# PSeitz/veloci

Hardware: AMD Instinct MI355X
Metric: queries/sec, 3-term AND on 100M-doc index (p50 latency and HBM fraction alongside) (higher is better)
Workload: dtype u32 doc ids + f16->f32 scores

## Files before the change

veloci_amd/csrc/scan_probe.hip:

```cpp
#include <hip/hip_runtime.h>
#include <hip/hip_fp16.h>

#include "device_types.hpp"
#include "kernel_common.hpp"
#include "kernels.hpp"
#include "probe_common.hpp"

namespace vq {

#ifdef VQ_STAMP
__device__ unsigned long long g_probe_stamp[16];
#define PS_INIT                                                      \
    unsigned long long _st0 = __builtin_amdgcn_s_memtime();          \
    const unsigned long long _t0 = _st0;                             \
    const unsigned long long _r0 = __builtin_amdgcn_s_memrealtime(); \
    unsigned long long _acc[16] = {0};
#define PS_AT(k)                                                \
    {                                                           \
        unsigned long long _st1 = __builtin_amdgcn_s_memtime(); \
        _acc[k] += _st1 - _st0;                                 \
        _st0 = _st1;                                            \
    }
#define PS_COUNT(k) _acc[k] += 1ull;
#define PS_FLUSH                                                                                             \
    _acc[14] = __builtin_amdgcn_s_memtime() - _t0;                        \
    _acc[15] = __builtin_amdgcn_s_memrealtime() - _r0;                \
    if (threadIdx.x == 0) {                                                                                  \
        _Pragma("unroll") for (int _k = 0; _k < 16; ++_k) if (_acc[_k]) atomicAdd(&g_probe_stamp[_k], _acc[_k]); \
    }
void debug_read_probe_stamps(unsigned long long* out, int reset) {
    (void)hipMemcpyFromSymbol(out, HIP_SYMBOL(g_probe_stamp), sizeof(unsigned long long) * 16);
    if (reset) {
        unsigned long long z[16] = {0};
        (void)hipMemcpyToSymbol(HIP_SYMBOL(g_probe_stamp), z, sizeof z);
    }
}
#else
#define PS_INIT
#define PS_AT(k)
#define PS_COUNT(k)
#define PS_FLUSH
#endif

constexpr uint32_t kPMaxR = 2;
constexpr uint32_t kPU = 256;
static_assert(kPU >= 256, "a round of 256 postings must fit the empty queue");
constexpr uint32_t kPR = 128;
constexpr uint32_t kPLdsShape = 8;
constexpr uint32_t kPLdsU = kPLdsShape + 24;
constexpr uint32_t kPLdsR = kPLdsU + kPU;
__host__ __device__ constexpr uint32_t probe_lds_tile(uint32_t nd) { return kPLdsR + (2 + nd) * kPR; }
__host__ __device__ constexpr uint32_t probe_lds_arr(uint32_t nd, uint32_t nb) { return probe_lds_tile(nd) + nb * (kPTW + kPRk); }
size_t scan_probe_lds_bytes(uint32_t cand_cap, uint32_t nd, uint32_t na, uint32_t arr_slot) {
    return (size_t)(probe_lds_arr(nd, nd - na) + na * arr_slot + 2 * cand_cap) * 4 + 16;
}

template <uint32_t ND, uint32_t NA, bool OR = false>
__device__ __forceinline__ void probe_body(const uint8_t* __restrict__ blob, const uint32_t span, const uint32_t q, const uint32_t cand_cap, const uint32_t arr_slot,
                                           unsigned long long* __restrict__ span_keys, unsigned long long* __restrict__ num_hits) {
    extern __shared__ __attribute__((aligned(16))) uint32_t lds[];
    const uint32_t lane = threadIdx.x;
    const VQ_CONST QHeader* H = as_const<QHeader>(blob);
    const VQ_CONST DList* gl = as_const<DList>(blob + H->off_lists);
    const VQ_CONST DOp* gops = as_const<DOp>(blob + H->off_ops);
    const VQ_CONST DProbe* P = as_const<DProbe>(blob + H->off_simple2);
    const uint32_t sflags = H->simple_flags;
    const uint32_t top_k = H->top_k;
    constexpr uint32_t n = ND + 1u;
    constexpr uint32_t NB = ND - NA;
    constexpr uint32_t NB1 = NB ? NB : 1u, NA1 = NA ? NA : 1u;
    PS_INIT

    unsigned long long* thr = reinterpret_cast<unsigned long long*>(lds);
    uint32_t* cand_n = lds + 2;
    uint32_t* sh = lds + kPLdsShape;
    uint32_t* uq = lds + kPLdsU;
    uint32_t* rq = lds + kPLdsR;
    uint32_t* tile = lds + probe_lds_tile(ND);
    uint32_t* rank = tile + NB * kPTW;
    uint32_t* arr = lds + probe_lds_arr(ND, NB);
    unsigned long long* cand = reinterpret_cast<unsigned long long*>(arr + NA * arr_slot);
    unsigned long long* const gthr = reinterpret_cast<unsigned long long*>(const_cast<uint8_t*>(blob) + offsetof(QHeader, gthr));
    CandState cs{cand, cand_n, thr, cand_cap, gthr};
    cs.upper = H->key_upper;
    uint32_t* const stat = H->stat_off ? lds + 4 : nullptr;
    uint8_t* const pool = H->off_pool ? const_cast<uint8_t*>(blob) + H->off_pool : nullptr;

    const uint32_t* ccov = nullptr;
    const uint32_t* cgdir = nullptr;
    const uint32_t* d_bitmap[NB1];
    const uint32_t* d_rank[NB1];
    const uint16_t* d_arr[NA1];
    const uint32_t* d_agd[NA1];
    {
        const uint32_t ck = (uint32_t)__ffs((int)((sflags >> 8) & 0xFu)) - 1u;
        const uint32_t am = (sflags >> 12) & 0xFu;
        uint32_t role_of[4] = {0u, 0u, 0u, 0u};
        uint32_t ib = 0, ia = NB;
#pragma unroll
        for (uint32_t k = 0; k < n; ++k) {
            const VQ_CONST DList& d = gl[gops[k].list_begin];
            if (k == ck) {
                ccov = P->leaf[k].cov32;
                cgdir = P->leaf[k].gdir;
                if (lane == 0) {
                    sh[kShCts] = __float_as_uint(d.term_score);
                    sh[kShPrunable] = (d.term_score > 0.0f && d.max_raw < 0x7C00u) ? 1u : 0u;
                }
            } else {
                const bool is_arr = ((am >> k) & 1u) != 0u;
                const uint32_t role = is_arr ? ia : ib;
#pragma unroll
                for (uint32_t j = 0; j < NB; ++j)
                    if (!is_arr && j == role) {
                        d_bitmap[j] = d.bitmap;
                        d_rank[j] = d.rank_dir;
                    }
#pragma unroll
                for (uint32_t a = 0; a < NA; ++a)
                    if (is_arr && NB + a == role) {
                        d_arr[a] = P->leaf[k].arr16;
                        d_agd[a] = P->leaf[k].gdir;
                    }
                if (lane == 0) {
                    const uint16_t mr = d.max_raw;
                    sh[kShTs + role] = __float_as_uint(d.term_score);
                    sh[kShVmax + role] = (d.term_score > 0.0f && mr < 0x7C00u) ? __float_as_uint(posting_value(d.term_score, mr)) : 0x7F800000u;
                    reinterpret_cast<unsigned long long*>(sh + kShScores)[role] = is_arr ? (unsigned long long)(uintptr_t)P->leaf[k].cov32 : (unsigned long long)(uintptr_t)d.scores;
                }
                role_of[k] = 1u + role;
                if (is_arr) ++ia;
                else ++ib;
            }
        }
        const KOp root(gops + n);
#pragma unroll
        for (uint32_t j = 0; j < n; ++j) {
            const uint32_t k = OR ? j : root.and_order(j);
            if (lane == 0) sh[kShSrc + j] = k == 0u ? role_of[0] : k == 1u ? role_of[1] : k == 2u ? role_of[2] : role_of[3];
        }
    }

    const uint32_t n_spans = H->n_spans;
    const unsigned long long range = (unsigned long long)(H->doc_hi - H->doc_lo);
    const uint32_t span_lo = span == 0 ? H->doc_lo : ((H->doc_lo + (uint32_t)(range * span / n_spans)) & ~(kPT - 1u));
    const uint32_t span_hi = span + 1 == n_spans ? H->doc_hi : ((H->doc_lo + (uint32_t)(range * (span + 1) / n_spans)) & ~(kPT - 1u));
    const uint32_t bitmap_base = H->bitmap_base;
    const uint32_t keys_base = H->keys_base;

    if (lane == 0) {
        *thr = __hip_atomic_load(gthr, __ATOMIC_RELAXED, __HIP_MEMORY_SCOPE_AGENT);
        *cand_n = 0;
        lds[4] = 0u;
    }
    __syncthreads();
    unsigned long long thr_seen = *thr;
    uint32_t raw_min = 0u;
    constexpr uint32_t kMasks = OR ? (1u << ND) : 1u;
    uint32_t rmin[kMasks];
    auto take_raw_min = [&](const float thr_f) {
        if (OR) {
#pragma unroll
            for (uint32_t m = 0; m < kMasks; ++m) rmin[m] = probe_raw_min<ND>(sh, thr_f, lane, m);
        } else raw_min = probe_raw_min<ND>(sh, thr_f, lane);
    };
    take_raw_min(__uint_as_float(unorder_f32((uint32_t)(thr_seen >> 32))));

    const u32x4 kSent = u32x4{0xFFFFFFFFu, 0xFFFFFFFFu, 0xFFFFFFFFu, 0xFFFFFFFFu};
    const VQ_GLOBAL u32x4* cc4 = as_global(reinterpret_cast<const u32x4*>(ccov));

    uint32_t un = 0, rn = 0;
    uint32_t ucnt = 0;
    unsigned long long hits = 0;
    unsigned long long g_prev = 0ull;

    const uint32_t t_first = (span_lo - bitmap_base) >> kProbeTileShift;
    const uint32_t t_end = span_hi > span_lo ? ((span_hi - 1u - bitmap_base) >> kProbeTileShift) + 1u : t_first;
    uint32_t dir_base = t_first;
    auto load_dir = [&](const uint32_t* g) { return as_global(g)[dir_base + lane < t_end ? dir_base + lane : t_end]; };
    uint32_t dirv = load_dir(cgdir);
    uint32_t adv[NA1];
#pragma unroll
    for (uint32_t a = 0; a < NA; ++a) adv[a] = load_dir(d_agd[a]);
    auto dir_at = [&](const uint32_t v, const uint32_t tt) { return (uint32_t)__builtin_amdgcn_readlane((int)v, (int)(tt - dir_base)); };

    u32x4 wk[ND][kPNV];
    uint32_t rk[NB1];
    u32x4 nid[kPMaxR], cid[kPMaxR];
#pragma unroll
    for (uint32_t r = 0; r < kPMaxR; ++r) nid[r] = cid[r] = kSent;
    uint32_t pf_rounds = 0, pf_v0 = 0, pf_v1 = 0;
    uint32_t na_g0[NA1], na_nv[NA1];
    uint32_t a_g0[NA1], a_cnt[NA1];
#pragma unroll
    for (uint32_t a = 0; a < NA1; ++a) na_g0[a] = na_nv[a] = a_g0[a] = a_cnt[a] = 0u;
    auto issue_tile = [&](const uint32_t tt, const uint32_t g0, const uint32_t g1) {
        pf_rounds = (g1 - g0 + 31u) >> 5;
        pf_v0 = g0 * 2u;
        pf_v1 = g1 * 2u;
        if (OR || pf_rounds) {
#pragma unroll
            for (uint32_t i = 0; i < NB; ++i) {
                const VQ_GLOBAL u32x4* gb = as_global(reinterpret_cast<const u32x4*>(d_bitmap[i] + (size_t)tt * kPTW));
#pragma unroll
                for (uint32_t h = 0; h < kPNV; ++h) wk[i][h] = gb[h * 64u + lane];
                rk[i] = as_global(d_rank[i])[tt * kPRk + lane];
            }
#pragma unroll
            for (uint32_t a = 0; a < NA; ++a) {
                const VQ_GLOBAL u32x4* ga = as_global(reinterpret_cast<const u32x4*>(d_arr[a]) + na_g0[a]);
#pragma unroll
                for (uint32_t h = 0; h < kPNV; ++h)
                    if (h * 64u + lane < na_nv[a]) wk[NB + a][h] = ga[h * 64u + lane];
            }
#pragma unroll
            for (uint32_t r = 0; r < kPMaxR; ++r) {
                const uint32_t v = pf_v0 + r * 64u + lane;
                nid[r] = kSent;
                if (r < pf_rounds && v < pf_v1) nid[r] = cc4[v];
            }
        }
    };

    uint32_t tile_lo = 0;
    uint32_t f_stage = 0;
    uint32_t f_doc = 0, f_idx[ND];
    float f_vc = 0.0f, f_vd[ND];
    uint16_t f_r = 0;
    bool f_alive = false;
#pragma unroll
    for (uint32_t i = 0; i < ND; ++i) {
        f_idx[i] = 0u;
        f_vd[i] = 0.0f;
    }
    uint32_t rhead = 0;
    uint32_t tiles_since_merge = 8;
    auto push_keys = [&](const unsigned long long key, bool pending, const bool final) {
        if (wballot(pending)) {
            while (true) {
                if (pending) {
                    if (key > *thr) {
                        uint32_t pos = atomicAdd(cs.n, 1u);
                        if (pos < cs.cap) {
                            cs.cand[pos] = key;
                            pending = false;
                        }
                    } else pending = false;
                }
                probe_lds_fence();
                if (!wballot(pending)) break;
                cand_prune(cs, top_k);
            }
            if (pool && (tiles_since_merge >= 8u || final)) {
                PS_COUNT(13)
                tiles_since_merge = 0;
                probe_pool_merge<true>(cs, top_k, pool, lane);
            }
            const unsigned long long tn = *thr;
            if ((uint32_t)(tn >> 32) != (uint32_t)(thr_seen >> 32)) take_raw_min(__uint_as_float(unorder_f32((uint32_t)(tn >> 32))));
            thr_seen = tn;
        }
    };
    uint32_t f_mask = 0;
    auto sum_of = [&](const ProbeShape<ND>& S, const float vc, const float (&vd)[ND], const uint32_t mask) { return OR ? probe_or_sum<ND>(S, vc, vd, mask) : probe_sum<ND>(S, vc, vd); };
    auto flush_final = [&](const ProbeShape<ND>& S, const bool final) {
        const float score = sum_of(S, f_vc, f_vd, f_mask);
        const unsigned long long key = ((unsigned long long)order_f32(__float_as_uint(score)) << 32) | (unsigned long long)f_doc;
        f_stage = 0;
        PS_COUNT(12)
        push_keys(key, f_alive && key > *thr && key < cs.upper, final);
    };
    auto flush_service = [&](const bool final) {
        const unsigned long long* sptr = reinterpret_cast<const unsigned long long*>(sh + kShScores);
        unsigned long long gp = sptr[0];
        uint32_t gidx = 0u;
        if (f_stage) {
            const ProbeShape<ND> S = probe_shape<ND>(sh);
            const float thr_f = __uint_as_float(unorder_f32((uint32_t)(*thr >> 32)));
            bool last = true;
#pragma unroll
            for (uint32_t i = 0; i < ND; ++i)
                if (f_stage == i + 1u) {
                    f_vd[i] = posting_value(S.ts[i], f_r);
                    if (i + 1u < ND) {
                        constexpr uint32_t zero = 0;
                        f_alive = f_alive && !(sum_of(S, f_vc, f_vd, f_mask) < thr_f);
                        if (stat && lane == 0) *stat += 2u * (uint32_t)__popcll(wballot(f_alive));
                        gp = sptr[i + 1u < ND ? i + 1u : zero];
                        gidx = (f_alive && (!OR || ((f_mask >> (i + 1u < ND ? i + 1u : zero)) & 1u))) ? f_idx[i + 1u < ND ? i + 1u : zero] : 0u;
                        last = false;
                    }
                }
            if (last) flush_final(S, final);
            else ++f_stage;
        } else if (rn >= 64u || (final && rn)) {
            const uint32_t count = rn < 64u ? rn : 64u;
            probe_lds_fence();
            f_alive = lane < count;
            uint32_t raw = 0;
            const uint32_t slot = (rhead + lane) & (kPR - 1u);
            if (f_alive) {
                f_doc = rq[slot];
                raw = rq[kPR + slot];
#pragma unroll
                for (uint32_t i = 0; i < ND; ++i) f_idx[i] = rq[(2u + i) * kPR + slot];
            }
            if (OR) {
                f_mask = 0u;
#pragma unroll
                for (uint32_t i = 0; i < ND; ++i) f_mask |= f_idx[i] != 0xFFFFFFFFu ? 1u << i : 0u;
            }
            f_vc = posting_value(__uint_as_float(sh[kShCts]), (uint16_t)raw);
#pragma unroll
            for (uint32_t i = 0; i < ND; ++i) f_vd[i] = __uint_as_float(sh[kShVmax + i]);
            if (stat && lane == 0) *stat += 2u * count;
            gidx = (f_alive && (!OR || (f_mask & 1u))) ? f_idx[0] : 0u;
            f_stage = 1u;
            rhead = (rhead + count) & (kPR - 1u);
            rn -= count;
        }
        f_r = as_global(reinterpret_cast<const uint16_t*>((uintptr_t)gp))[gidx];
    };
    auto flush_sync = [&]() {
        const ProbeShape<ND> S = probe_shape<ND>(sh);
        probe_lds_fence();
        const uint32_t slot = (rhead + lane) & (kPR - 1u);
        const uint32_t doc = rq[slot];
        const float vc = posting_value(S.cts, (uint16_t)rq[kPR + slot]);
        float vd[ND];
        uint32_t mask = 0;
#pragma unroll
        for (uint32_t i = 0; i < ND; ++i) {
            const uint16_t* sp = reinterpret_cast<const uint16_t*>((uintptr_t) reinterpret_cast<const unsigned long long*>(sh + kShScores)[i]);
            const uint32_t ix = rq[(2u + i) * kPR + slot];
            if (ix != 0xFFFFFFFFu) mask |= 1u << i;
            vd[i] = posting_value(S.ts[i], as_global(sp)[(OR && ix == 0xFFFFFFFFu) ? 0u : ix]);
        }
        if (stat && lane == 0) *stat += 2u * ND * 64u;
        const float score = sum_of(S, vc, vd, mask);
        const unsigned long long key = ((unsigned long long)order_f32(__float_as_uint(score)) << 32) | (unsigned long long)doc;
        rhead = (rhead + 64u) & (kPR - 1u);
        rn -= 64u;
        push_keys(key, key > *thr && key < cs.upper, false);
    };
    auto bitmap_rank = [&](const uint32_t i, const uint32_t rel) {
        const uint32_t g = rel >> kRankShift, wi = (rel >> 5) & 15u, below = (1u << (rel & 31u)) - 1u;
        const int full = (int)((1u << wi) - 1u);
        const uint32_t* tl = tile + i * kPTW;
        uint32_t acc = rank[i * kPRk + g] + (uint32_t)__popc(tl[rel >> 5] & below);
        const u32x4* gw = reinterpret_cast<const u32x4*>(tl + g * 16u);
#pragma unroll
        for (uint32_t v4 = 0; v4 < 4; ++v4) {
            const u32x4 x = gw[v4];
            acc += (uint32_t)__popc(x.x & (uint32_t)__builtin_amdgcn_sbfe(full, v4 * 4u + 0u, 1u));
            acc += (uint32_t)__popc(x.y & (uint32_t)__builtin_amdgcn_sbfe(full, v4 * 4u + 1u, 1u));
            acc += (uint32_t)__popc(x.z & (uint32_t)__builtin_amdgcn_sbfe(full, v4 * 4u + 2u, 1u));
            acc += (uint32_t)__popc(x.w & (uint32_t)__builtin_amdgcn_sbfe(full, v4 * 4u + 3u, 1u));
        }
        return acc;
    };
    auto rank_some = [&](const uint32_t cnt) {
        while (rn + cnt > kPR) flush_sync();
        probe_lds_fence();
        const uint32_t* const uqe = uq + (un - cnt);
        un -= cnt;
        if (NA == 0u && ND == 2u && cnt <= 32u) {
            const uint32_t el = lane & 31u, role = lane >> 5;
            if (el < cnt) {
                const uint32_t e = uqe[el];
                const uint32_t rel = e >> 16;
                const uint32_t slot = (rhead + rn + el) & (kPR - 1u);
                if (role == 0u) {
                    rq[slot] = tile_lo + rel;
                    rq[kPR + slot] = e & 0xFFFFu;
                }
                const bool here = !OR || ((tile[role * kPTW + (rel >> 5)] >> (rel & 31u)) & 1u) != 0u;
                rq[(2u + role) * kPR + slot] = here ? bitmap_rank(role, rel) : 0xFFFFFFFFu;
            }
            rn += cnt;
        } else if (NA == 0u) {
            if (lane < cnt) {
                const uint32_t e = uqe[lane];
                const uint32_t rel = e >> 16;
                const uint32_t slot = (rhead + rn + lane) & (kPR - 1u);
                rq[slot] = tile_lo + rel;
                rq[kPR + slot] = e & 0xFFFFu;
#pragma unroll
                for (uint32_t i = 0; i < NB; ++i) {
                    const bool here = !OR || ((tile[i * kPTW + (rel >> 5)] >> (rel & 31u)) & 1u) != 0u;
                    rq[(2u + i) * kPR + slot] = here ? bitmap_rank(i, rel) : 0xFFFFFFFFu;
                }
            }
            rn += cnt;
        } else {
            uint32_t e = 0xFFFFFFFFu, pos[NA1];
            bool found = lane < cnt;
            if (found) e = uqe[lane];
            const uint32_t rel = e >> 16;
#pragma unroll
            for (uint32_t a = 0; a < NA; ++a) {
                const uint16_t* A = reinterpret_cast<const uint16_t*>(arr + a * arr_slot);
                uint32_t lo = 0u, len = a_cnt[a];
#ifdef VQ_PROBE_NO_SEARCH
                lo = rel & 7u;
                len = 0u;
#endif
                while (len > 1u) {
                    const uint32_t half = len >> 1;
                    lo = (uint32_t)A[lo + half] <= rel ? lo + half : lo;
                    len -= half;
                }
#ifdef VQ_PROBE_NO_SEARCH
                found = found && a_cnt[a] != 0u && ((uint32_t)A[lo] ^ rel) < 0x2000u;
#else
                found = found && a_cnt[a] != 0u && (uint32_t)A[lo] == rel;
#endif
                pos[a] = lo;
            }
            const unsigned long long fm = wballot(found);
            hits += (unsigned long long)__popcll(fm);
            const bool live = found && (e & 0xFFFFu) >= raw_min;
            const unsigned long long lm = wballot(live);
            if (lm) {
                if (live) {
                    const uint32_t slot = (rhead + rn + (uint32_t)__popcll(lm & ((1ull << lane) - 1ull))) & (kPR - 1u);
                    rq[slot] = tile_lo + rel;
                    rq[kPR + slot] = e & 0xFFFFu;
#pragma unroll
                    for (uint32_t i = 0; i < NB; ++i) rq[(2u + i) * kPR + slot] = bitmap_rank(i, rel);
#pragma unroll
                    for (uint32_t a = 0; a < NA; ++a) rq[(2u + NB + a) * kPR + slot] = (a_g0[a] * 8u + pos[a]) * 2u;
                }
                rn += (uint32_t)__popcll(lm);
            }
        }
    };
    uint32_t lo_rel = 0, width = 0;
    struct ProbeWords {
        uint32_t w[OR ? ND : 1u][4];
    };
    auto probe_read = [&](const u32x4 e4) {
        const uint32_t ee[4] = {e4.x, e4.y, e4.z, e4.w};
        ProbeWords pw;
#pragma unroll
        for (uint32_t c = 0; c < 4; ++c) {
            const uint32_t a = (ee[c] >> 21) & (kPTW - 1u);
            if (OR) {
#pragma unroll
                for (uint32_t i = 0; i < ND; ++i) pw.w[OR ? i : 0u][c] = tile[i * kPTW + a];
            } else {
                pw.w[0][c] = 0xFFFFFFFFu;
                if (NB) {
                    pw.w[0][c] = tile[a];
#pragma unroll
                    for (uint32_t i = 1; i < NB; ++i) pw.w[0][c] &= tile[i * kPTW + a];
                }
            }
        }
        return pw;
    };
    auto probe_eval = [&](const u32x4 e4, const ProbeWords& pw, const bool may_overflow) {
        const uint32_t ee[4] = {e4.x, e4.y, e4.z, e4.w};
        unsigned long long lm[4];
        bool live[4];
#pragma unroll
        for (uint32_t c = 0; c < 4; ++c) {
            const uint32_t rel = ee[c] >> 16;
            const bool in = (rel - lo_rel) < width;
            if (OR) {
                uint32_t mask = 0;
#pragma unroll
                for (uint32_t i = 0; i < ND; ++i) mask |= ((pw.w[OR ? i : 0u][c] >> (rel & 31u)) & 1u) << i;
                uint32_t need = rmin[0];
#pragma unroll
                for (uint32_t m = 1; m < kMasks; ++m) need = mask == m ? rmin[OR ? m : 0u] : need;
                hits += (unsigned long long)__popcll(wballot(in && mask == 0u));
                live[c] = in && (ee[c] & 0xFFFFu) >= need;
                lm[c] = wballot(live[c]);
                continue;
            }
            const bool bit = ((pw.w[0][c] >> (rel & 31u)) & 1u) != 0u;
            const unsigned long long sm = NB ? (wballot(in) & wballot(bit)) : wballot(in);
            if (NA == 0u) {
                const bool strong = (ee[c] & 0xFFFFu) >= raw_min;
                hits += (unsigned long long)__popcll(sm);
                lm[c] = sm & wballot(strong);
                live[c] = in && bit && strong;
            } else {
                lm[c] = sm;
                live[c] = in && bit;
            }
        }
        if (lm[0] | lm[1] | lm[2] | lm[3]) {
            if (may_overflow) {
                const uint32_t add = (uint32_t)__popcll(lm[0]) + (uint32_t)__popcll(lm[1]) + (uint32_t)__popcll(lm[2]) + (uint32_t)__popcll(lm[3]);
                while (un + add > kPU) rank_some(un < 64u ? un : 64u);
            }
#pragma unroll
            for (uint32_t c = 0; c < 4; ++c) {
                if (live[c]) uq[un + (uint32_t)__popcll(lm[c] & ((1ull << lane) - 1ull))] = ee[c];
                un += (uint32_t)__popcll(lm[c]);
            }
        }
    };

    uint32_t t = t_first;
    tile_lo = bitmap_base + (t_first << kProbeTileShift);
    auto next_arrays = [&](const uint32_t tt) {
#pragma unroll
        for (uint32_t a = 0; a < NA; ++a) {
            na_g0[a] = dir_at(adv[a], tt);
            na_nv[a] = dir_at(adv[a], tt + 1u) - na_g0[a];
        }
    };
    if (t < t_end) {
        next_arrays(t);
        issue_tile(t, dir_at(dirv, t), dir_at(dirv, t + 1u));
    }
    PS_AT(0)
    while (t < t_end) {
        PS_COUNT(8)
        __builtin_amdgcn_s_waitcnt(0x0F70);
        __builtin_amdgcn_s_setprio(3);
        const uint32_t rounds = pf_rounds, v0 = pf_v0, v1 = pf_v1;
        if (OR || rounds) {
            if (OR) {
#pragma unroll
                for (uint32_t h = 0; h < kPNV; ++h) {
                    u32x4 u = wk[0][h];
#pragma unroll
                    for (uint32_t i = 1; i < NB; ++i) u |= wk[i][h];
                    ucnt += (uint32_t)__popc(u.x) + (uint32_t)__popc(u.y) + (uint32_t)__popc(u.z) + (uint32_t)__popc(u.w);
                }
            }
#pragma unroll
            for (uint32_t i = 0; i < NB; ++i) {
#pragma unroll
                for (uint32_t h = 0; h < kPNV; ++h) reinterpret_cast<u32x4*>(tile + i * kPTW)[h * 64u + lane] = wk[i][h];
                rank[i * kPRk + lane] = rk[i];
            }
#pragma unroll
            for (uint32_t a = 0; a < NA; ++a) {
#pragma unroll
                for (uint32_t h = 0; h < kPNV; ++h)
                    if (h * 64u + lane < na_nv[a]) reinterpret_cast<u32x4*>(arr + a * arr_slot)[h * 64u + lane] = wk[NB + a][h];
                a_g0[a] = na_g0[a];
                a_cnt[a] = na_nv[a] * 8u;
            }
#pragma unroll
            for (uint32_t r = 0; r < kPMaxR; ++r) {
                cid[r] = nid[r];
                asm volatile("" : "+v"(cid[r]));
            }
        }
        {
            uint32_t fr = f_r, glo = (uint32_t)g_prev, ghi = (uint32_t)(g_prev >> 32);
            asm volatile("" : "+v"(fr), "+v"(glo), "+v"(ghi), "+v"(dirv));
#pragma unroll
            for (uint32_t a = 0; a < NA; ++a) asm volatile("" : "+v"(adv[a]));
            f_r = (uint16_t)fr;
            g_prev = ((unsigned long long)ghi << 32) | glo;
        }
        PS_AT(1)
        if (lane == 0 && g_prev > *thr) *thr = g_prev;
        const bool more = t + 1u < t_end;
        uint32_t ng0 = 0, ng1 = 0;
        if (more) {
            if (t + 2u - dir_base >= 64u) {
                dir_base = t + 1u;
                dirv = load_dir(cgdir);
#pragma unroll
                for (uint32_t a = 0; a < NA; ++a) adv[a] = load_dir(d_agd[a]);
            }
            ng0 = dir_at(dirv, t + 1u);
            ng1 = dir_at(dirv, t + 2u);
            next_arrays(t + 1u);
        }
        if (f_stage || rn >= 64u) PS_COUNT(11)
        flush_service(false);
        PS_AT(4)
        if (more) issue_tile(t + 1u, ng0, ng1);
        else pf_rounds = 0;
        if (lane == 0) g_prev = __hip_atomic_load(gthr, __ATOMIC_RELAXED, __HIP_MEMORY_SCOPE_AGENT);
        __builtin_amdgcn_s_setprio(0);
        probe_lds_fence();
        {
            const unsigned long long tn = *thr;
            if ((uint32_t)(tn >> 32) != (uint32_t)(thr_seen >> 32)) take_raw_min(__uint_as_float(unorder_f32((uint32_t)(tn >> 32))));
            thr_seen = tn;
            ++tiles_since_merge;
        }
        PS_AT(5)
#ifdef VQ_PROBE_STREAM_ONLY
        hits += (unsigned long long)__popcll(wballot((cid[0].x ^ cid[1].y) == 0x12345u));
        if (rounds && span == 0xFFFFFFFFu) {
#else
        if (rounds) {
#endif
            const uint32_t tile_end = tile_lo + kPT;
            const uint32_t tile_hi = (tile_end > tile_lo && tile_end < span_hi) ? tile_end : span_hi;
            const uint32_t lo_bound = tile_lo > span_lo ? tile_lo : span_lo;
            lo_rel = lo_bound - tile_lo;
            width = tile_hi - lo_bound;
            {
                ProbeWords pw[kPMaxR];
#pragma unroll
                for (uint32_t r = 0; r < kPMaxR; ++r)
                    if (r < rounds) pw[r] = probe_read(cid[r]);
#pragma unroll
                for (uint32_t r = 0; r < kPMaxR; ++r)
                    if (r < rounds) {
                        PS_COUNT(9)
                        probe_eval(cid[r], pw[r], r > 0u);
                    }
            }
            for (uint32_t r = kPMaxR; r < rounds; ++r) {
                const uint32_t v = v0 + r * 64u + lane;
                u32x4 e4 = kSent;
                if (v < v1) e4 = cc4[v];
                PS_COUNT(9)
                const ProbeWords pw = probe_read(e4);
                probe_eval(e4, pw, true);
            }
            PS_AT(2)
            while (un) {
                PS_COUNT(10)
                rank_some(un < 64u ? un : 64u);
            }
            PS_AT(3)
        }
        ++t;
        tile_lo += kPT;
    }
    while (f_stage || rn) flush_service(true);
    __syncthreads();
    cand_prune(cs, top_k);
    {
        const uint32_t cn = *cand_n;
        unsigned long long* out = span_keys + (size_t)keys_base + (size_t)span * top_k;
        for (uint32_t i = lane; i < top_k; i += 64u) out[i] = i < cn ? cand[i] : 0ull;
    }
    if (OR) {
        uint32_t total;
        (void)wave_excl_scan_u32(ucnt, &total);
        hits += (unsigned long long)total;
    }
    if (lane == 0 && hits) atomicAdd(&num_hits[q], hits);
    if (lane == 0 && H->stat_off && lds[4]) atomicAdd(&num_hits[H->stat_off], (unsigned long long)lds[4]);
    PS_AT(6)
    PS_FLUSH
}

__device__ __forceinline__ void probe_item(const uint32_t* __restrict__ span_base, const uint32_t* __restrict__ qmap, uint32_t nq, uint32_t* q, uint32_t* span) {
    uint32_t lo = 0, hi = nq;
    const uint32_t wg = blockIdx.x;
    while (hi - lo > 1) {
        uint32_t mid = (lo + hi) >> 1;
        if (span_base[mid] <= wg) lo = mid;
        else hi = mid;
    }
    *span = blockIdx.x - span_base[lo];
    *q = qmap[lo];
}

#define VQ_PROBE_PARAMS                                                                                                                                       \
    const uint8_t *__restrict__ blobs, const uint32_t *__restrict__ blob_off, const uint32_t *__restrict__ span_base, const uint32_t *__restrict__ qmap, uint32_t nq, \
        uint32_t cand_cap, uint32_t arr_slot, unsigned long long *__restrict__ span_keys, unsigned long long *__restrict__ num_hits
#define VQ_PROBE_ITEM                           \
    uint32_t q, span;                           \
    probe_item(span_base, qmap, nq, &q, &span); \
    const uint8_t* blob = blobs + blob_off[q];
#ifndef VQ_PROBE_WAVES
#define VQ_PROBE_WAVES 4
#endif
#define VQ_PROBE_KERNEL(waves) __global__ __launch_bounds__(64) __attribute__((amdgpu_waves_per_eu(waves, 8))) void

VQ_PROBE_KERNEL(VQ_PROBE_WAVES) k_scan_probe_1(VQ_PROBE_PARAMS) {
    VQ_PROBE_ITEM
    if (((as_const<QHeader>(blob)->simple_flags >> 12) & 0xFu) == 0u) probe_body<1, 0>(blob, span, q, cand_cap, arr_slot, span_keys, num_hits);
    else probe_body<1, 1>(blob, span, q, cand_cap, arr_slot, span_keys, num_hits);
}
VQ_PROBE_KERNEL(VQ_PROBE_WAVES) k_scan_probe_2_0(VQ_PROBE_PARAMS) {
    VQ_PROBE_ITEM
    probe_body<2, 0>(blob, span, q, cand_cap, arr_slot, span_keys, num_hits);
}
VQ_PROBE_KERNEL(VQ_PROBE_WAVES) k_scan_probe_2_1(VQ_PROBE_PARAMS) {
    VQ_PROBE_ITEM
    probe_body<2, 1>(blob, span, q, cand_cap, arr_slot, span_keys, num_hits);
}
VQ_PROBE_KERNEL(VQ_PROBE_WAVES) k_scan_probe_2_2(VQ_PROBE_PARAMS) {
    VQ_PROBE_ITEM
    probe_body<2, 2>(blob, span, q, cand_cap, arr_slot, span_keys, num_hits);
}
VQ_PROBE_KERNEL(3) k_scan_probe_3_0(VQ_PROBE_PARAMS) {
    VQ_PROBE_ITEM
    probe_body<3, 0>(blob, span, q, cand_cap, arr_slot, span_keys, num_hits);
}
VQ_PROBE_KERNEL(3) k_scan_probe_3_1(VQ_PROBE_PARAMS) {
    VQ_PROBE_ITEM
    probe_body<3, 1>(blob, span, q, cand_cap, arr_slot, span_keys, num_hits);
}
VQ_PROBE_KERNEL(3) k_scan_probe_3_2(VQ_PROBE_PARAMS) {
    VQ_PROBE_ITEM
    probe_body<3, 2>(blob, span, q, cand_cap, arr_slot, span_keys, num_hits);
}
VQ_PROBE_KERNEL(3) k_scan_probe_3_3(VQ_PROBE_PARAMS) {
    VQ_PROBE_ITEM
    probe_body<3, 3>(blob, span, q, cand_cap, arr_slot, span_keys, num_hits);
}

VQ_PROBE_KERNEL(3) k_scan_probe_or(VQ_PROBE_PARAMS) {
    VQ_PROBE_ITEM
    if (as_const<QHeader>(blob)->simple_n == 2u) probe_body<1, 0, true>(blob, span, q, cand_cap, arr_slot, span_keys, num_hits);
    else probe_body<2, 0, true>(blob, span, q, cand_cap, arr_slot, span_keys, num_hits);
}

static auto* probe_kernel(uint32_t shape) {
    return shape == kProbeAnd1 ? k_scan_probe_1 : shape == kProbeAnd2A0 ? k_scan_probe_2_0 : shape == kProbeAnd2A1 ? k_scan_probe_2_1 : shape == kProbeAnd2A2 ? k_scan_probe_2_2 :
           shape == kProbeAnd3A0 ? k_scan_probe_3_0 : shape == kProbeAnd3A1 ? k_scan_probe_3_1 : shape == kProbeAnd3A2 ? k_scan_probe_3_2 : shape == kProbeAnd3A3 ? k_scan_probe_3_3 :
                                                                                                                                                                    k_scan_probe_or;
}

uint32_t debug_probe_occupancy(uint32_t shape, size_t lds_bytes) {
    int n = 0;
    if (shape >= kProbeShapes || hipOccupancyMaxActiveBlocksPerMultiprocessor(&n, probe_kernel(shape), 64, lds_bytes) != hipSuccess || n < 0) return 0;
    return (uint32_t)n;
}

void launch_scan_probe_shape(hipStream_t st, uint32_t shape, uint32_t na_seen, uint32_t arr_slot, uint32_t total_spans, const uint8_t* blobs, const uint32_t* blob_off,
                             const uint32_t* span_base, const uint32_t* qmap, uint32_t nq, uint32_t cand_cap, unsigned long long* span_keys, unsigned long long* num_hits) {
    if (!total_spans) return;
    const uint32_t nd = shape == kProbeAnd1 ? 1u : (shape >= kProbeAnd3A0 && shape <= kProbeAnd3A3) ? 3u : 2u;
    size_t lds = 0;
    for (uint32_t na = 0; na <= nd; ++na)
        if ((na_seen >> na) & 1u) lds = std::max(lds, scan_probe_lds_bytes(cand_cap, nd, na, arr_slot));
    hipLaunchKernelGGL(probe_kernel(shape), dim3(total_spans), dim3(64), lds, st, blobs, blob_off, span_base, qmap, nq, cand_cap, arr_slot, span_keys, num_hits);
}

}
```

Before: 164,800.

## Scalarize base pointers, branchless LDS binary search, streamline probe evaluation

Forces the per-term base pointers to scalar registers with readfirstlane so global loads use scalar bases plus a lane offset. It replaces the LDS binary search over array containers with a fixed-depth, scalar-stepped search, and folds the span-range test into the rank stage. It also rewrites the AND path of probe_eval to compact each column with mbcnt. Overflow checks now use a precomputed posting bound instead of a popcount sum. These cut VALU and address arithmetic in the hot probe loop. The trade-off is a conservative overflow bound that may flush more often, plus subtle correctness dependencies on the new pass predicate.

Measured after the change: 166,700 (median of 6 runs). Within noise of the previous version (+1.1%).

```diff
diff --git a/veloci_amd/csrc/scan_probe.hip b/veloci_amd/csrc/scan_probe.hip
--- a/veloci_amd/csrc/scan_probe.hip
+++ b/veloci_amd/csrc/scan_probe.hip
@@ -41,6 +41,21 @@
 #define PS_COUNT(k)
 #define PS_FLUSH
 #endif
+
+__device__ __forceinline__ uint32_t lanes_below(const unsigned long long m, const uint32_t base) {
+    return __builtin_amdgcn_mbcnt_hi((uint32_t)(m >> 32), __builtin_amdgcn_mbcnt_lo((uint32_t)m, base));
+}
+
+template <class T>
+__device__ __forceinline__ const T* uniform_ptr(const T* p) {
+    uint32_t lo = (uint32_t)__builtin_amdgcn_readfirstlane((int)(uint32_t)(uintptr_t)p), hi = (uint32_t)__builtin_amdgcn_readfirstlane((int)(uint32_t)((uintptr_t)p >> 32));
+    asm volatile("" : "+s"(lo), "+s"(hi));
+    return reinterpret_cast<const T*>(((uintptr_t)hi << 32) | (uintptr_t)lo);
+}
+template <class T>
+__device__ __forceinline__ const VQ_GLOBAL T* uniform_base(const T* p) {
+    return as_global(uniform_ptr(p));
+}
 
 constexpr uint32_t kPMaxR = 2;
 constexpr uint32_t kPU = 256;
@@ -141,6 +156,19 @@
         }
     }
 
+    ccov = uniform_ptr(ccov);
+    cgdir = uniform_ptr(cgdir);
+#pragma unroll
+    for (uint32_t i = 0; i < NB; ++i) {
+        d_bitmap[i] = uniform_ptr(d_bitmap[i]);
+        d_rank[i] = uniform_ptr(d_rank[i]);
+    }
+#pragma unroll
+    for (uint32_t a = 0; a < NA; ++a) {
+        d_arr[a] = uniform_ptr(d_arr[a]);
+        d_agd[a] = uniform_ptr(d_agd[a]);
+    }
+
     const uint32_t n_spans = H->n_spans;
     const unsigned long long range = (unsigned long long)(H->doc_hi - H->doc_lo);
     const uint32_t span_lo = span == 0 ? H->doc_lo : ((H->doc_lo + (uint32_t)(range * span / n_spans)) & ~(kPT - 1u));
@@ -192,8 +220,12 @@
     uint32_t pf_rounds = 0, pf_v0 = 0, pf_v1 = 0;
     uint32_t na_g0[NA1], na_nv[NA1];
     uint32_t a_g0[NA1], a_cnt[NA1];
-#pragma unroll
-    for (uint32_t a = 0; a < NA1; ++a) na_g0[a] = na_nv[a] = a_g0[a] = a_cnt[a] = 0u;
+    int32_t na_left[NA1];
+#pragma unroll
+    for (uint32_t a = 0; a < NA1; ++a) {
+        na_g0[a] = na_nv[a] = a_g0[a] = a_cnt[a] = 0u;
+        na_left[a] = 0;
+    }
     auto issue_tile = [&](const uint32_t tt, const uint32_t g0, const uint32_t g1) {
         pf_rounds = (g1 - g0 + 31u) >> 5;
         pf_v0 = g0 * 2u;
@@ -201,23 +233,23 @@
         if (OR || pf_rounds) {
 #pragma unroll
             for (uint32_t i = 0; i < NB; ++i) {
-                const VQ_GLOBAL u32x4* gb = as_global(reinterpret_cast<const u32x4*>(d_bitmap[i] + (size_t)tt * kPTW));
+                const VQ_GLOBAL u32x4* gb = uniform_base(reinterpret_cast<const u32x4*>(d_bitmap[i] + (size_t)tt * kPTW));
 #pragma unroll
                 for (uint32_t h = 0; h < kPNV; ++h) wk[i][h] = gb[h * 64u + lane];
-                rk[i] = as_global(d_rank[i])[tt * kPRk + lane];
+                rk[i] = uniform_base(d_rank[i] + (size_t)tt * kPRk)[lane];
             }
 #pragma unroll
             for (uint32_t a = 0; a < NA; ++a) {
-                const VQ_GLOBAL u32x4* ga = as_global(reinterpret_cast<const u32x4*>(d_arr[a]) + na_g0[a]);
+                const VQ_GLOBAL u32x4* ga = uniform_base(reinterpret_cast<const u32x4*>(d_arr[a]) + na_g0[a]);
 #pragma unroll
                 for (uint32_t h = 0; h < kPNV; ++h)
-                    if (h * 64u + lane < na_nv[a]) wk[NB + a][h] = ga[h * 64u + lane];
-            }
+                    if (na_left[a] > (int32_t)(h * 64u)) wk[NB + a][h] = ga[h * 64u + lane];
+            }
+            const VQ_GLOBAL u32x4* gc = uniform_base(reinterpret_cast<const u32x4*>(ccov) + pf_v0);
 #pragma unroll
             for (uint32_t r = 0; r < kPMaxR; ++r) {
-                const uint32_t v = pf_v0 + r * 64u + lane;
                 nid[r] = kSent;
-                if (r < pf_rounds && v < pf_v1) nid[r] = cc4[v];
+                if (r < pf_rounds && r * 64u + lane < pf_v1 - pf_v0) nid[r] = gc[r * 64u + lane];
             }
         }
     };
@@ -349,16 +381,23 @@
         const uint32_t* tl = tile + i * kPTW;
         uint32_t acc = rank[i * kPRk + g] + (uint32_t)__popc(tl[rel >> 5] & below);
         const u32x4* gw = reinterpret_cast<const u32x4*>(tl + g * 16u);
+        auto below_word = [&](const uint32_t x, const uint32_t j) {
+            uint32_t m = (uint32_t)__builtin_amdgcn_sbfe(full, j, 1u);
+            if (NA != 0u) asm volatile("" : "+v"(m));
+            acc += (uint32_t)__popc(x & m);
+            if (NA != 0u) asm volatile("" : "+v"(acc));
+        };
 #pragma unroll
         for (uint32_t v4 = 0; v4 < 4; ++v4) {
             const u32x4 x = gw[v4];
-            acc += (uint32_t)__popc(x.x & (uint32_t)__builtin_amdgcn_sbfe(full, v4 * 4u + 0u, 1u));
-            acc += (uint32_t)__popc(x.y & (uint32_t)__builtin_amdgcn_sbfe(full, v4 * 4u + 1u, 1u));
-            acc += (uint32_t)__popc(x.z & (uint32_t)__builtin_amdgcn_sbfe(full, v4 * 4u + 2u, 1u));
-            acc += (uint32_t)__popc(x.w & (uint32_t)__builtin_amdgcn_sbfe(full, v4 * 4u + 3u, 1u));
+            below_word(x.x, v4 * 4u + 0u);
+            below_word(x.y, v4 * 4u + 1u);
+            below_word(x.z, v4 * 4u + 2u);
+            below_word(x.w, v4 * 4u + 3u);
         }
         return acc;
     };
+    uint32_t lo_rel = 0, width = 0;
     auto rank_some = [&](const uint32_t cnt) {
         while (rn + cnt > kPR) flush_sync();
         probe_lds_fence();
@@ -397,6 +436,7 @@
             bool found = lane < cnt;
             if (found) e = uqe[lane];
             const uint32_t rel = e >> 16;
+            found = found && (rel - lo_rel) < width;
 #pragma unroll
             for (uint32_t a = 0; a < NA; ++a) {
                 const uint16_t* A = reinterpret_cast<const uint16_t*>(arr + a * arr_slot);
@@ -405,11 +445,22 @@
                 lo = rel & 7u;
                 len = 0u;
 #endif
-                while (len > 1u) {
-                    const uint32_t half = len >> 1;
-                    lo = (uint32_t)A[lo + half] <= rel ? lo + half : lo;
-                    len -= half;
-                }
+#ifndef VQ_PROBE_NO_SEARCH
+                if (len > 1u) {
+                    const uint32_t top = 31u - (uint32_t)__clz((int)len);
+                    typedef const __attribute__((address_space(3))) uint16_t* LdsU16;
+                    const LdsU16 A0 = (LdsU16)A;
+                    LdsU16 w = A0 + len - (1u << top);
+                    w = (uint32_t)w[0] <= rel ? w : A0;
+                    uint32_t steps = (1u << top) - 1u;
+#pragma unroll
+                    for (int k = 11; k >= 0; --k) {
+                        asm volatile("" : "+s"(steps));
+                        if ((steps >> k) & 1u) w = (uint32_t)w[1u << k] <= rel ? w + (1u << k) : w;
+                    }
+                    lo = (uint32_t)(w - A0);
+                }
+#endif
 #ifdef VQ_PROBE_NO_SEARCH
                 found = found && a_cnt[a] != 0u && ((uint32_t)A[lo] ^ rel) < 0x2000u;
 #else
@@ -423,7 +474,7 @@
             const unsigned long long lm = wballot(live);
             if (lm) {
                 if (live) {
-                    const uint32_t slot = (rhead + rn + (uint32_t)__popcll(lm & ((1ull << lane) - 1ull))) & (kPR - 1u);
+                    const uint32_t slot = lanes_below(lm, rhead + rn) & (kPR - 1u);
                     rq[slot] = tile_lo + rel;
                     rq[kPR + slot] = e & 0xFFFFu;
 #pragma unroll
@@ -435,7 +486,6 @@
             }
         }
     };
-    uint32_t lo_rel = 0, width = 0;
     struct ProbeWords {
         uint32_t w[OR ? ND : 1u][4];
     };
@@ -459,15 +509,15 @@
         }
         return pw;
     };
-    auto probe_eval = [&](const u32x4 e4, const ProbeWords& pw, const bool may_overflow) {
+    auto probe_eval = [&](const u32x4 e4, const ProbeWords& pw, const uint32_t behind) {
         const uint32_t ee[4] = {e4.x, e4.y, e4.z, e4.w};
-        unsigned long long lm[4];
-        bool live[4];
-#pragma unroll
-        for (uint32_t c = 0; c < 4; ++c) {
-            const uint32_t rel = ee[c] >> 16;
-            const bool in = (rel - lo_rel) < width;
-            if (OR) {
+        if (OR) {
+            unsigned long long lm[4];
+            bool live[4];
+#pragma unroll
+            for (uint32_t c = 0; c < 4; ++c) {
+                const uint32_t rel = ee[c] >> 16;
+                const bool in = (rel - lo_rel) < width;
                 uint32_t mask = 0;
 #pragma unroll
                 for (uint32_t i = 0; i < ND; ++i) mask |= ((pw.w[OR ? i : 0u][c] >> (rel & 31u)) & 1u) << i;
@@ -477,30 +527,38 @@
                 hits += (unsigned long long)__popcll(wballot(in && mask == 0u));
                 live[c] = in && (ee[c] & 0xFFFFu) >= need;
                 lm[c] = wballot(live[c]);
-                continue;
-            }
-            const bool bit = ((pw.w[0][c] >> (rel & 31u)) & 1u) != 0u;
-            const unsigned long long sm = NB ? (wballot(in) & wballot(bit)) : wballot(in);
-            if (NA == 0u) {
-                const bool strong = (ee[c] & 0xFFFFu) >= raw_min;
-                hits += (unsigned long long)__popcll(sm);
-                lm[c] = sm & wballot(strong);
-                live[c] = in && bit && strong;
-            } else {
-                lm[c] = sm;
-                live[c] = in && bit;
-            }
-        }
-        if (lm[0] | lm[1] | lm[2] | lm[3]) {
-            if (may_overflow) {
-                const uint32_t add = (uint32_t)__popcll(lm[0]) + (uint32_t)__popcll(lm[1]) + (uint32_t)__popcll(lm[2]) + (uint32_t)__popcll(lm[3]);
-                while (un + add > kPU) rank_some(un < 64u ? un : 64u);
-            }
-#pragma unroll
-            for (uint32_t c = 0; c < 4; ++c) {
-                if (live[c]) uq[un + (uint32_t)__popcll(lm[c] & ((1ull << lane) - 1ull))] = ee[c];
-                un += (uint32_t)__popcll(lm[c]);
-            }
+            }
+            if (lm[0] | lm[1] | lm[2] | lm[3]) {
+                if (behind) {
+                    const uint32_t add = (uint32_t)__popcll(lm[0]) + (uint32_t)__popcll(lm[1]) + (uint32_t)__popcll(lm[2]) + (uint32_t)__popcll(lm[3]);
+                    while (un + add > kPU) rank_some(un < 64u ? un : 64u);
+                }
+#pragma unroll
+                for (uint32_t c = 0; c < 4; ++c) {
+                    if (live[c]) uq[lanes_below(lm[c], un)] = ee[c];
+                    un += (uint32_t)__popcll(lm[c]);
+                }
+            }
+            return;
+        }
+        if (behind) {
+            while (un + behind > kPU) rank_some(un < 64u ? un : 64u);
+        }
+#pragma unroll
+        for (uint32_t c = 0; c < 4; ++c) {
+            const uint32_t rel = ee[c] >> 16;
+            bool live;
+            {
+                const uint32_t bit = NB ? (uint32_t)__builtin_amdgcn_sbfe((int)pw.w[0][c], rel & 31u, 1u) : 0xFFFFFFFFu;
+                const bool pass = NA ? (bit & 0x80000000u) > ee[c] : (rel - lo_rel) < (bit & width);
+                if (NA == 0u) {
+                    hits += (unsigned long long)__popcll(wballot(pass));
+                    live = pass && (ee[c] & 0xFFFFu) >= raw_min;
+                } else live = pass;
+            }
+            const unsigned long long m = wballot(live);
+            if (live) uq[lanes_below(m, un)] = ee[c];
+            un += (uint32_t)__popcll(m);
         }
     };
 
@@ -511,6 +569,8 @@
         for (uint32_t a = 0; a < NA; ++a) {
             na_g0[a] = dir_at(adv[a], tt);
             na_nv[a] = dir_at(adv[a], tt + 1u) - na_g0[a];
+            na_left[a] = (int32_t)(na_nv[a] - lane);
+            asm volatile("" : "+v"(na_left[a]));
         }
     };
     if (t < t_end) {
@@ -543,7 +603,7 @@
             for (uint32_t a = 0; a < NA; ++a) {
 #pragma unroll
                 for (uint32_t h = 0; h < kPNV; ++h)
-                    if (h * 64u + lane < na_nv[a]) reinterpret_cast<u32x4*>(arr + a * arr_slot)[h * 64u + lane] = wk[NB + a][h];
+                    if (na_left[a] > (int32_t)(h * 64u)) reinterpret_cast<u32x4*>(arr + a * arr_slot)[h * 64u + lane] = wk[NB + a][h];
                 a_g0[a] = na_g0[a];
                 a_cnt[a] = na_nv[a] * 8u;
             }
@@ -602,6 +662,7 @@
             const uint32_t lo_bound = tile_lo > span_lo ? tile_lo : span_lo;
             lo_rel = lo_bound - tile_lo;
             width = tile_hi - lo_bound;
+            const auto round_postings = [&](const uint32_t r) { return (v1 - v0 - r * 64u < 64u ? v1 - v0 - r * 64u : 64u) * 4u; };
             {
                 ProbeWords pw[kPMaxR];
 #pragma unroll
@@ -611,7 +672,7 @@
                 for (uint32_t r = 0; r < kPMaxR; ++r)
                     if (r < rounds) {
                         PS_COUNT(9)
-                        probe_eval(cid[r], pw[r], r > 0u);
+                        probe_eval(cid[r], pw[r], r ? round_postings(r) : 0u);
                     }
             }
             for (uint32_t r = kPMaxR; r < rounds; ++r) {
@@ -620,7 +681,7 @@
                 if (v < v1) e4 = cc4[v];
                 PS_COUNT(9)
                 const ProbeWords pw = probe_read(e4);
-                probe_eval(e4, pw, true);
+                probe_eval(e4, pw, round_postings(r));
             }
             PS_AT(2)
             while (un) {
```
